# TencentARC/ViT-Lens

Measured on AMD Instinct MI355X. Metric: modality-pairs/sec (ViT-L, 224^2 patches), higher is better.
Workload: dtype bf16; 1 GPU; C3: ViT-L Lens(depth)->ViT + image + text tri-modal InfoNCE TRAINING step (fwd+bwd+AdamW), batch 1024/GPU in micro-batches of 256, first 4 blocks + adapter trainable; global_batch=1024, residual_dtype=bf16, accumulate=fp32, parallelism=dp1, gemm_cfg=-1, via=step, text_tower_operands=fp16, layernorm=folded into the GEMMs (frozen blocks), frozen_towers=second HIP stream beside the trainable tower's forward, backward=two halves of the micro-batches on two HIP streams

## Files before the change

include/vitlens_hip.h:

```cpp
#ifndef VITLENS_HIP_H
#define VITLENS_HIP_H

#include <stdint.h>

#ifdef __cplusplus
extern "C" {
#endif

#ifndef __HIP_PLATFORM_AMD__
typedef struct ihipStream_t* hipStream_t;
#endif

#define VL_EPI_BF16 0
#define VL_EPI_F32 1
#define VL_EPI_RES_F32 2
#define VL_EPI_RES_BF16 3
#define VL_EPI_GEGLU 5
#define VL_EPI_DGELU 6
#define VL_EPI_DGEGLU 7
#define VL_ACT_NONE 0
#define VL_ACT_GELU 1
#define VL_ACT_RELU 2
#define VL_ACT_GELU_DSAVE 4

#define VL_F32 0
#define VL_BF16 1
#define VL_F16 2

#define VL_GEMM_AUTO (-1)
#define VL_GEMM_PERSIST 8
#define VL_GEMM_PINGPONG 10

const char* vl_last_error(void);
#define VL_ABI_VERSION 601
int vl_version(void);

int vl_gemm_bf16(const void* A, const void* W, const float* bias, void* out, const void* res,
                 int M, int N, int K, int lda, int ldw, int ldo, float alpha, int epi, int act,
                 int cfg, hipStream_t stream);

int vl_gemm_splitk_accum_f32(const void* A, const void* W, float* out, int M, int N, int K, int lda, int ldw, long ldo,
                             float alpha, int splits, float* ws, hipStream_t stream);
int vl_gemm_tn_splitk_accum_f32(const void* At, const void* Bt, float* out, int M, int N, int K, int lda, int ldb, long ldo,
                                float alpha, int splits, float* ws, hipStream_t stream);
int vl_gemm_bf16_ex(const void* A, const void* W, const float* bias, void* out, const void* res, void* out2,
                    int M, int N, int K, int lda, int ldw, int ldo, float alpha, int epi, int act,
                    int res_div, int cfg, hipStream_t stream);

int vl_gemm_f16(const void* A, const void* W, const float* bias, void* out, const void* res, int M, int N, int K,
                int lda, int ldw, int ldo, float alpha, int epi, int act, hipStream_t stream);
int vl_attn_fwd_f16(const void* q, const void* k, const void* v, const long* strides, void* out, float* lse,
                    int B, int H, int Lq, int Lk, int dh, float qscale, int causal, hipStream_t stream);

int vl_gemm_f32(const float* A, const float* W, const float* bias, float* out, const float* res, int M, int N, int K,
                int lda, int ldw, int ldo, float alpha, int act, hipStream_t stream);
int vl_attn_fwd_f32(const float* q, const float* k, const float* v, const long* strides, float* out, float* lse,
                    int B, int H, int Lq, int Lk, int dh, float scale, int causal, hipStream_t stream);
int vl_im2col_f32(const float* x, float* patches, int N, int C, int H, int W, int kh, int kw, int sh, int sw,
                  int Kp, int transpose_hw, hipStream_t stream);

int vl_device_info(int device, char* arch, int arch_len, int* cus, int* clock_khz, long* hbm_bytes);

int vl_attn_fwd_bf16(const void* q, const void* k, const void* v, const long* strides, void* out, float* lse,
                     int B, int H, int Lq, int Lk, int dh, float qscale, int causal, hipStream_t stream);

int vl_gemm_main_rows(int M, int N);
int vl_gemm_lnfold_bf16(const void* A, const void* Wg, const float* bias_f, const float* ln_c, const float* ln_mean,
                        const float* ln_rstd, void* out, void* out2, int M, int N, int K, int lda, int ldw, int ldo, int act,
                        hipStream_t stream);
int vl_gemm_res_rowstats_bf16(const void* A, const void* W, const float* bias, void* out, const void* res, float* row_part,
                              int M, int N, int K, int lda, int ldw, int ldo, hipStream_t stream);
int vl_ln_row_stats(const float* row_part, int P, const void* x_bf16, long x_row_stride, int D, int m_main, int rows, float eps,
                    float* mean, float* rstd, const float* ln_w, const float* ln_b, void* y_left, long y_row_stride, int y_row0,
                    hipStream_t stream);

int vl_layernorm_fwd(const void* x, int x_dtype, long x_row_stride, const int64_t* row_index, long row_mul,
                     const float* w, const float* b, void* y, int y_dtype, long y_row_stride,
                     float* mean, float* rstd, int rows, int D, float eps, hipStream_t stream);

int vl_assemble_ln_pre(const void* tokens, int tok_dtype, const float* cls, const float* pos, const float* pos2,
// ... 114 lines not shown
```

vit-lens_amd/csrc/vl_gemm.hip:

```cpp
#include "vl_gemm_common.h"

namespace {

template <int EPI, int MT, int NTL>
__device__ __forceinline__ void store_tile(const GemmP& p, f32x16 (&acc)[MT][NTL], int mrow0, int ncol0, int fr, int fg) {
#pragma unroll
  for (int i = 0; i < MT; ++i) {
    const int m = mrow0 + i * 32 + fr;
    if (m >= p.M) continue;
#pragma unroll
    for (int j = 0; j < NTL; ++j) {
#pragma unroll
      for (int q = 0; q < 4; ++q) {
        const int n = ncol0 + j * 32 + q * 8 + fg * 4;
        if (n >= p.N) continue;
        float v[4];
#pragma unroll
        for (int e = 0; e < 4; ++e) v[e] = acc[i][j][q * 4 + e] * p.alpha;
        if (p.bias) {
          const f32x4 bv = *(const f32x4*)(p.bias + n);
#pragma unroll
          for (int e = 0; e < 4; ++e) v[e] += bv[e];
        }
        if constexpr (EPI == EPI_BF16) {
// ... 598 lines not shown
  }
}

static int query_cus() {
  int dev = 0, n = 0;
  if (hipGetDevice(&dev) != hipSuccess || hipDeviceGetAttribute(&n, hipDeviceAttributeMultiprocessorCount, dev) != hipSuccess || n <= 0) n = 256;
  return n;
}
static int num_cus() {
  static const int n = query_cus();
  return n;
}

template <int EPI, int BN = 256, int NWAVES = 8>
hipError_t launch_persist(const GemmP& p, hipStream_t s) {
  using S = Smem<256, BN>;
  constexpr int WM = NWAVES == 4 ? 2 : (BN == 256 ? 2 : 4), WN = NWAVES / WM;
  const int tiles = ((p.M + 255) / 256) * ((p.N + BN - 1) / BN);
  auto kern = gemm_nt_persist2_kernel<256, BN, WM, WN, EPI>;
  constexpr int smem = 2 * S::STAGE + 8 * 4096;
  static const hipError_t attr = hipFuncSetAttribute((const void*)kern, hipFuncAttributeMaxDynamicSharedMemorySize, smem);
  if (attr != hipSuccess) return attr;
  int G = num_cus() & ~7;
  if (tiles < G) G = (tiles + 7) & ~7;
  hipLaunchKernelGGL(kern, dim3(G), dim3(NWAVES * 64), smem, s, p);
  return hipGetLastError();
}

}
bool vl_gemm_park_supported(int epi, const void* params);
int vl_gemm_park_launch(int epi, const void* params, int ncu, hipStream_t s);
bool vl_gemm_pp_supported(int epi, const void* params);
int vl_gemm_pp_launch(int epi, const void* params, int ncu, hipStream_t s);
namespace {

template <int EPI>
hipError_t launch_best_persist(const GemmP& p0, hipStream_t s) {
  const GemmP& p = p0;
  if (vl_gemm_park_supported(EPI, &p)) return (hipError_t)vl_gemm_park_launch(EPI, &p, num_cus(), s);
  if (vl_gemm_pp_supported(EPI, &p)) return (hipError_t)vl_gemm_pp_launch(EPI, &p, num_cus(), s);
  return launch_persist<EPI>(p, s);
}

template <int EPI>
hipError_t dispatch(const GemmP& p, int cfg, hipStream_t s) {
  if (cfg == 8) {
    if (!vl_gemm_park_supported(EPI, &p)) return hipErrorInvalidValue;
    return (hipError_t)vl_gemm_park_launch(EPI, &p, num_cus(), s);
  }
  if (cfg == 10) {
    if (!vl_gemm_pp_supported(EPI, &p)) return hipErrorInvalidValue;
    return (hipError_t)vl_gemm_pp_launch(EPI, &p, num_cus(), s);
  }
  if (cfg == 4 || cfg == 5) return launch_persist<EPI>(p, s);
  if (cfg == 6) return launch_persist<EPI, 128>(p, s);
  if (cfg == 9) return launch_tail<EPI>(p, s);
  if (cfg == 11) return launch<64, 64, 2, 2, EPI, true>(p, s);
  if (cfg == 12) return launch<128, 64, 2, 2, EPI, true>(p, s);
  switch (cfg & 3) {
    case 0: return launch<256, 256, 2, 4, EPI, true>(p, s);
    case 1: return launch<128, 128, 2, 2, EPI, true>(p, s);
    case 2: return launch<256, 256, 2, 4, EPI, false>(p, s);
    default: return launch<128, 128, 2, 2, EPI, false>(p, s);
  }
}

}

extern "C" int vl_set_error(const char* msg);

static int gcd_i(int a, int b) { while (b) { int t = a % b; a = b; b = t; } return a; }

template <int EPI>
static hipError_t run_gemm(const GemmP& p, int cfg, hipStream_t s) {
  if (cfg >= 0) return dispatch<EPI>(p, cfg, s);
  const int G = num_cus() & ~7;
  const int tiles_n = (p.N + 255) / 256, full_m = p.M / 256;
  if ((long)full_m * tiles_n < (G * 3) / 4) return dispatch<EPI>(p, 1, s);
  int step = G / gcd_i(G, tiles_n);
  int main_m = (full_m / step) * step;
  if ((p.N & 255) == 128) {
    step = 2 * G / gcd_i(2 * G, p.N >> 7);
    main_m = (full_m / step) * step;
    if (main_m == 0) main_m = full_m;
  }
  if (main_m == 0) main_m = full_m;
  if (main_m == 0) return launch_persist<EPI>(p, s);
  const int rows_main = main_m * 256;
  GemmP pm = p; pm.M = rows_main;
  hipError_t e = launch_best_persist<EPI>(pm, s);
  if (e != hipSuccess || rows_main == p.M) return e;
  GemmP pr = p;
  pr.M = p.M - rows_main; pr.m_off = p.m_off + rows_main;
  pr.A = p.A + (size_t)rows_main * p.lda;
  constexpr size_t osz = (EPI == EPI_F32 || EPI == EPI_RES_F32) ? 4 : 2;
  if (p.out) pr.out = (unsigned char*)p.out + (size_t)rows_main * p.ldo * osz;
  if (p.res && EPI != EPI_RES_BF16) pr.res = (const unsigned char*)p.res + (size_t)rows_main * p.ldo * osz;
  if (p.out2) pr.out2 = (bf16_t*)p.out2 + (size_t)rows_main * p.ldo * (EPI == EPI_GEGLU ? 2 : 1);
  if (pr.M > 512) return dispatch<EPI>(pr, 1, s);
  const long t64 = (long)((pr.M + 63) / 64) * ((pr.N + 63) / 64);
  return t64 >= 192 ? dispatch<EPI>(pr, 11, s) : launch_tail<EPI>(pr, s);
}

#define VL_CHECK_ARG(c, msg) do { if (!(c)) return vl_set_error(msg); } while (0)

extern "C" int vl_gemm_main_rows(int M, int N) {
  const int G = num_cus() & ~7;
  if (M <= 0 || N <= 0 || (N & 255)) return 0;
  const int tiles_n = N / 256, full_m = M / 256;
  if ((long)full_m * tiles_n < (G * 3) / 4) return 0;
  const int step = G / gcd_i(G, tiles_n);
  int main_m = (full_m / step) * step;
  if (main_m == 0) main_m = full_m;
  return main_m * 256;
}

extern "C" int vl_gemm_lnfold_bf16(const void* A, const void* Wg, const float* bias_f, const float* ln_c, const float* ln_mean,
                                   const float* ln_rstd, void* out, void* out2, int M, int N, int K, int lda, int ldw, int ldo,
                                   int act, hipStream_t stream) {
  VL_CHECK_ARG(A && Wg && bias_f && ln_c && ln_mean && ln_rstd && out, "vl_gemm_lnfold_bf16: null operand");
  VL_CHECK_ARG(act == VL_ACT_NONE || act == VL_ACT_GELU || act == VL_ACT_GELU_DSAVE, "vl_gemm_lnfold_bf16: act must be none, GELU or GELU_DSAVE");
  VL_CHECK_ARG((act == VL_ACT_GELU_DSAVE) == (out2 != nullptr), "vl_gemm_lnfold_bf16: out2 goes with VL_ACT_GELU_DSAVE");
  VL_CHECK_ARG((((uintptr_t)ln_c | (uintptr_t)bias_f) & 15) == 0, "vl_gemm_lnfold_bf16: column vectors must be 16-byte aligned");
  GemmP p{};
  p.A = (const bf16_t*)A; p.W = (const bf16_t*)Wg; p.bias = bias_f; p.out = out; p.out2 = out2;
  p.M = M; p.N = N; p.K = K; p.lda = lda; p.ldw = ldw; p.ldo = ldo; p.alpha = 1.0f; p.act = act; p.res_div = 1;
  p.ln_mean = ln_mean; p.ln_rstd = ln_rstd; p.ln_c = ln_c;
  const GemmP& q = p;
  VL_CHECK_ARG(vl_gemm_park_supported(EPI_BF16, &q), "vl_gemm_lnfold_bf16: whole 256x256 tiles, K >= 512, 16-byte aligned operands required");
  const hipError_t e = (hipError_t)vl_gemm_park_launch(EPI_BF16, &q, num_cus(), stream);
  if (e != hipSuccess) return vl_set_error(hipGetErrorString(e));
  return 0;
}

extern "C" int vl_gemm_res_rowstats_bf16(const void* A, const void* W, const float* bias, void* out, const void* res,
                                         float* row_part, int M, int N, int K, int lda, int ldw, int ldo, hipStream_t stream) {
  VL_CHECK_ARG(A && W && out && res && row_part, "vl_gemm_res_rowstats_bf16: null operand");
  VL_CHECK_ARG((((uintptr_t)row_part) & 7) == 0, "vl_gemm_res_rowstats_bf16: row_part must be 8-byte aligned");
  GemmP p{};
  p.A = (const bf16_t*)A; p.W = (const bf16_t*)W; p.bias = bias; p.out = out; p.res = res;
  p.M = M; p.N = N; p.K = K; p.lda = lda; p.ldw = ldw; p.ldo = ldo; p.alpha = 1.0f; p.res_div = 1;
  p.row_part = row_part;
  const GemmP& q = p;
  VL_CHECK_ARG(vl_gemm_park_supported(EPI_RES_BF16, &q), "vl_gemm_res_rowstats_bf16: whole 256x256 tiles, K >= 512, 16-byte aligned operands required");
  const hipError_t e = (hipError_t)vl_gemm_park_launch(EPI_RES_BF16, &q, num_cus(), stream);
  if (e != hipSuccess) return vl_set_error(hipGetErrorString(e));
  return 0;
}

extern "C" int vl_gemm_bf16_ex(const void* A, const void* W, const float* bias, void* out, const void* res, void* out2,
                               int M, int N, int K, int lda, int ldw, int ldo, float alpha, int epi, int act,
                               int res_div, int cfg, hipStream_t stream);
extern "C" int vl_gemm_bf16(const void* A, const void* W, const float* bias, void* out, const void* res,
                            int M, int N, int K, int lda, int ldw, int ldo, float alpha, int epi, int act,
                            int cfg, hipStream_t stream) {
  return vl_gemm_bf16_ex(A, W, bias, out, res, nullptr, M, N, K, lda, ldw, ldo, alpha, epi, act, 1, cfg, stream);
}

extern "C" int vl_gemm_bf16_ex(const void* A, const void* W, const float* bias, void* out, const void* res, void* out2,
                               int M, int N, int K, int lda, int ldw, int ldo, float alpha, int epi, int act,
                               int res_div, int cfg, hipStream_t stream) {
  VL_CHECK_ARG(res_div >= 1, "vl_gemm_bf16: res_div must be >= 1");
  VL_CHECK_ARG(res_div == 1 || epi == VL_EPI_RES_BF16, "vl_gemm_bf16: row-broadcast residual needs VL_EPI_RES_BF16");
  VL_CHECK_ARG(M > 0 && N > 0 && K > 0, "vl_gemm_bf16: empty problem");
  VL_CHECK_ARG((K & 63) == 0, "vl_gemm_bf16: K must be a multiple of 64");
  VL_CHECK_ARG((N & 3) == 0, "vl_gemm_bf16: N must be a multiple of 4");
  VL_CHECK_ARG((lda & 7) == 0 && (ldw & 7) == 0, "vl_gemm_bf16: lda/ldw must be multiples of 8");
  VL_CHECK_ARG((ldo & 3) == 0, "vl_gemm_bf16: ldo must be a multiple of 4");
  GemmP p{};
  p.A = (const bf16_t*)A; p.W = (const bf16_t*)W; p.bias = bias; p.out = out; p.res = res; p.out2 = out2;
  p.M = M; p.N = N; p.K = K; p.lda = lda; p.ldw = ldw; p.ldo = ldo; p.alpha = alpha; p.act = act; p.res_div = res_div;
  hipError_t e;
  switch (epi) {
    case VL_EPI_BF16:
      VL_CHECK_ARG(act != VL_ACT_GELU_DSAVE || out2, "vl_gemm_bf16: VL_ACT_GELU_DSAVE needs out2 (the gelu' tensor)");
      e = run_gemm<EPI_BF16>(p, cfg, stream); break;
    case VL_EPI_F32: e = run_gemm<EPI_F32>(p, cfg, stream); break;
    case VL_EPI_RES_F32: VL_CHECK_ARG(res, "vl_gemm_bf16: residual missing"); e = run_gemm<EPI_RES_F32>(p, cfg, stream); break;
    case VL_EPI_RES_BF16: VL_CHECK_ARG(res, "vl_gemm_bf16: residual missing"); e = run_gemm<EPI_RES_BF16>(p, cfg, stream); break;
    case VL_EPI_GEGLU: e = run_gemm<EPI_GEGLU>(p, cfg, stream); break;
    case VL_EPI_DGELU: VL_CHECK_ARG(res, "vl_gemm_bf16: pre-activation tensor missing"); e = run_gemm<EPI_DGELU>(p, cfg, stream); break;
    case VL_EPI_DGEGLU: VL_CHECK_ARG(res, "vl_gemm_bf16: pre-activation tensor missing"); VL_CHECK_ARG((ldo & 7) == 0, "vl_gemm_bf16: DGEGLU needs ldo % 8 == 0"); e = run_gemm<EPI_DGEGLU>(p, cfg, stream); break;
    default: return vl_set_error("vl_gemm_bf16: unknown epilogue");
  }
  if (e != hipSuccess) return vl_set_error(hipGetErrorString(e));
  return 0;
}

extern "C" int vl_gemm_f16(const void* A, const void* W, const float* bias, void* out, const void* res, int M, int N, int K,
                           int lda, int ldw, int ldo, float alpha, int epi, int act, hipStream_t stream) {
  VL_CHECK_ARG(A && W && out, "vl_gemm_f16: null operand");
  VL_CHECK_ARG(epi == VL_EPI_BF16 || epi == VL_EPI_RES_F32, "vl_gemm_f16: VL_EPI_BF16 (16-bit output, here fp16) or VL_EPI_RES_F32");
  VL_CHECK_ARG(epi != VL_EPI_RES_F32 || (res && act == VL_ACT_NONE), "vl_gemm_f16: VL_EPI_RES_F32 needs res and takes no activation");
  VL_CHECK_ARG(act == VL_ACT_NONE || act == VL_ACT_GELU, "vl_gemm_f16: act must be none or GELU");
  GemmP p{};
  p.A = (const bf16_t*)A; p.W = (const bf16_t*)W; p.bias = bias; p.out = out; p.res = res;
  p.M = M; p.N = N; p.K = K; p.lda = lda; p.ldw = ldw; p.ldo = ldo; p.alpha = alpha; p.act = act; p.res_div = 1; p.f16 = 1;
  const int e_ = epi == VL_EPI_BF16 ? (int)EPI_BF16 : (int)EPI_RES_F32;
  VL_CHECK_ARG(vl_gemm_park_supported(e_, &p), "vl_gemm_f16: whole 256x256 tiles (M % 256 == N % 256 == 0), K % 64 == 0, K >= 512, 16-byte aligned operands required");
  const hipError_t e = (hipError_t)vl_gemm_park_launch(e_, &p, num_cus(), stream);
  if (e != hipSuccess) return vl_set_error(hipGetErrorString(e));
  return 0;
}

bool vl_gemm_tn_supported(const void* params);
int vl_gemm_tn_launch(const void* params, int ncu, hipStream_t s);

extern "C" int vl_gemm_tn_splitk_accum_f32(const void* At, const void* Bt, float* out, int M, int N, int K, int lda, int ldb,
                                           long ldo, float alpha, int splits, float* ws, hipStream_t stream) {
  VL_CHECK_ARG(M > 0 && N > 0 && K > 0, "vl_gemm_tn_splitk: empty problem");
  VL_CHECK_ARG((M & 255) == 0 && (N & 255) == 0 && (K & 63) == 0, "vl_gemm_tn_splitk: M % 256, N % 256, K % 64 required");
  VL_CHECK_ARG((lda & 7) == 0 && (ldb & 7) == 0 && (ldo & 3) == 0 && lda >= M && ldb >= N, "vl_gemm_tn_splitk: lda/ldb % 8, ldo % 4, lda >= M, ldb >= N required");
  VL_CHECK_ARG(splits >= 1 && splits <= 1024 && ws, "vl_gemm_tn_splitk: 1 <= splits <= 1024 and a workspace of splits*M*N floats");
  const int nk = K >> 6;
  const int len = (nk + splits - 1) / splits, eff = (nk + len - 1) / len;
// ... 52 lines not shown
```

vit-lens_amd/vitlens_hip/_lib.py:

```python
import ctypes as C
import os

_HERE = os.path.dirname(os.path.abspath(__file__))
_LIB = None


class LibraryNotBuilt(ImportError):
    pass


def lib_path() -> str:
    return os.path.join(_HERE, "libvitlens_hip.so")


P, I, L, F = C.c_void_p, C.c_int, C.c_long, C.c_float

ABI_VERSION = 601

SIGNATURES = {
    "vl_version": [],
    "vl_device_info": [I, C.c_char_p, I, C.POINTER(I), C.POINTER(I), C.POINTER(L)],
    "vl_gemm_bf16": [P, P, P, P, P, I, I, I, I, I, I, F, I, I, I, P],
    "vl_gemm_splitk_accum_f32": [P, P, P, I, I, I, I, I, L, F, I, P, P],
    "vl_gemm_tn_splitk_accum_f32": [P, P, P, I, I, I, I, I, L, F, I, P, P],
    "vl_attn_fwd_bf16": [P, P, P, P, P, P, I, I, I, I, I, F, I, P],
    "vl_gemm_f16": [P, P, P, P, P, I, I, I, I, I, I, F, I, I, P],
    "vl_gemm_f32": [P, P, P, P, P, I, I, I, I, I, I, F, I, P],
    "vl_attn_fwd_f32": [P, P, P, P, P, P, I, I, I, I, I, F, I, P],
    "vl_im2col_f32": [P, P, I, I, I, I, I, I, I, I, I, I, P],
    "vl_attn_fwd_f16": [P, P, P, P, P, P, I, I, I, I, I, F, I, P],
    "vl_layernorm_fwd": [P, I, L, P, L, P, P, P, I, L, P, P, I, I, F, P],
    "vl_gemm_main_rows": [I, I],
    "vl_gemm_lnfold_bf16": [P, P, P, P, P, P, P, P, I, I, I, I, I, I, I, P],
    "vl_gemm_res_rowstats_bf16": [P, P, P, P, P, P, I, I, I, I, I, I, P],
    "vl_ln_row_stats": [P, I, P, L, I, I, I, F, P, P, P, P, P, L, I, P],
    "vl_assemble_ln_pre": [P, I, P, P, P, P, P, P, I, P, P, P, I, I, I, F, P],
    "vl_l2_normalize": [P, P, P, P, I, I, F, P],
    "vl_l2_normalize_bwd": [P, P, P, P, I, I, F, P],
    "vl_im2col_bf16": [P, P, I, I, I, I, I, I, I, I, I, I, P],
    "vl_text_embed": [P, P, P, P, I, I, I, I, I, P],
    "vl_cast_f32_bf16": [P, P, L, P],
    "vl_add_rows": [P, I, P, P, I, L, I, I, P],
    "vl_transpose_to_bf16": [P, I, L, I, I, P, L, P],
    "vl_transpose_colsum_bf16": [P, I, L, I, I, P, L, P, F, P, P],
    "vl_split_bf16x3": [P, P, L, I, I, P],
    "vl_ce_stats": [P, L, I, I, I, P, P, P, P, P],
    "vl_ce_loss_accum": [P, P, P, I, I, I, F, F, P, P],
    "vl_ce_grad": [P, L, I, I, I, P, P, F, F, P, L, P, L, F, P, P, P],
    "vl_ce_grad_ws_floats": [I, I, L, L],
    "vl_gemm_bf16_ex": [P, P, P, P, P, P, I, I, I, I, I, I, F, I, I, I, I, P],
    "vl_kaldi_fbank": [P, L, I, L, P, P, P, I, I, I, I, I, F, F, F, P],
    "vl_fps": [P, P, P, P, I, I, I, P],
    "vl_pc_gather_normalize": [P, P, P, I, I, I, I, P],
    "vl_resample_h_u8": [P, L, I, I, I, I, P, P, I, I, I, P, P],
    "vl_resample_v_u8_norm": [P, I, I, I, I, P, P, I, I, I, P, P, P, P, P],
    "vl_resample_batch_u8_norm": [P, I, I, I, I, I, P, P, P, P, P, P],
    "vl_resample_h_f32": [P, L, I, I, I, P, P, I, I, I, I, F, F, F, P, P],
    "vl_resample_v_f32_norm": [P, I, I, I, P, P, I, I, I, F, F, P, P],
    "vl_knn_group": [P, P, P, P, I, I, I, I, I, P],
    "vl_ball_group": [P, P, P, P, P, I, I, I, I, F, I, I, P],
    "vl_group_max": [P, L, P, I, L, L, I, I, P],
    "vl_pad3_bf16": [P, P, L, I, P],
    "vl_bn_stats": [P, L, I, I, P, I, P, P, P, P, F, P],
    "vl_bn_stats_local": [P, L, I, I, P, I, P, P],
    "vl_bn_stats_merge": [P, I, I, P, P, P, P, F, P, P],
    "vl_bn_bwd_reduce": [P, L, P, L, P, P, P, P, F, I, P, I, P, P, P, I, I, P],
    "vl_bn_bwd_apply": [P, L, P, L, P, P, P, P, F, I, P, P, P, L, I, I, P],
    "vl_bn_apply": [P, L, P, P, P, P, F, I, P, L, L, I, P],
    "vl_bn_bwd": [P, L, P, L, P, P, P, P, F, I, I, P, I, P, P, P, L, I, I, P],
    "vl_group_max_bwd": [P, L, P, L, P, L, P, L, L, I, I, P],
    "vl_group_sum": [P, L, P, L, L, I, I, P],
    "vl_layernorm_bwd": [P, I, L, P, I, L, P, P, P, P, P, P, L, I, I, P],
    "vl_layernorm_bwd_g": [P, I, L, P, I, L, P, P, P, P, P, I, P, L, I, I, P],
    "vl_colreduce_ws_floats": [I, I, I],
    "vl_layernorm_bwd_params": [P, I, L, P, I, L, P, P, P, P, I, I, P, P],
    "vl_colsum": [P, I, L, P, I, I, F, P, P],
    "vl_gelu_bf16": [P, P, L, P],
    "vl_geglu_bf16": [P, P, L, I, P],
    "vl_attn_bwd_bf16": [P, P, P, P, P, P, P, P, P, P, P, L, L, I, I, I, I, I, F, I, F, P],
    "vl_attn_bwd_fused_supported": [I, I, I, I],
    "vl_attn_bwd_fused_bf16": [P, P, P, P, P, P, P, P, P, P, L, L, I, I, I, I, F, F, P],
    "vl_adamw_step": [P, P, P, P, L, F, F, F, F, F, I, F, P],
    "vl_clamp_scalar": [P, F, F, P],
    "vl_axpy_f32": [P, P, F, L, P],
    "vl_scale_exp_f32": [P, P, L, P, F, P],
    "vl_batch_rowsum": [P, P, I, I, I, L, L, P],
    "vl_comm_unique_id": [P],
    "vl_comm_create": [C.POINTER(P), P, I, I],
    "vl_comm_destroy": [P],
    "vl_allgather_embed": [P, P, P, L, P],
    "vl_reducescatter_grad": [P, P, P, L, P],
    "vl_allreduce_grad": [P, P, L, P],
}


_RET = {"vl_colreduce_ws_floats": L, "vl_ce_grad_ws_floats": L}


def load_library():
    global _LIB
    if _LIB is not None:
        return _LIB
    path = lib_path()
    if not os.path.exists(path):
        raise LibraryNotBuilt(
            f"{path} is missing: build it with `python -c 'import __graft_entry__ as g; g.build()'` "
            "or `make -C vit-lens_amd/csrc` (hipcc --offload-arch=gfx950). No CPU/eager fallback exists.")
    lib = C.CDLL(path)
    lib.vl_last_error.restype = C.c_char_p
    lib.vl_last_error.argtypes = []
    for name, args in SIGNATURES.items():
        fn = getattr(lib, name)
        fn.argtypes = args
        fn.restype = _RET.get(name, I)
    got = int(lib.vl_version())
    if got != ABI_VERSION:
        raise RuntimeError(f"{path} reports ABI version {got}, this binding was written for {ABI_VERSION} "
                           "(include/vitlens_hip.h: VL_ABI_VERSION): rebuild the library (`make -C vit-lens_amd/csrc`)")
    _LIB = lib
    return lib


def check(status: int):
    if status != 0:
        raise RuntimeError("libvitlens_hip: " + load_library().vl_last_error().decode())
```

vit-lens_amd/vitlens_hip/ops.py:

```python
import ctypes as C
import threading

import torch

from ._lib import load_library, check

F32, BF16, F16 = 0, 1, 2
EPI_BF16, EPI_F32, EPI_RES_F32, EPI_RES_BF16, EPI_GEGLU, EPI_DGELU, EPI_DGEGLU = 0, 1, 2, 3, 5, 6, 7
ACT_NONE, ACT_GELU, ACT_RELU = 0, 1, 2
ACT_GELU_DSAVE = 4
LOG2E = 1.4426950408889634

_lib = load_library()


def _stream():
    return C.c_void_p(torch.cuda.current_stream().cuda_stream)


def _p(t):
    if t is None:
        return None
    if not t.is_cuda:
        raise RuntimeError("vitlens_hip ops need GPU tensors (no CPU fallback)")
# ... 14 lines not shown
    if t.dim() != 2 or t.stride(1) != 1:
        raise ValueError(f"{name}: need a row-major 2-D tensor, got shape {tuple(t.shape)} strides {t.stride()}")
    if dtype is not None and t.dtype != dtype:
        raise TypeError(f"{name}: expected {dtype}, got {t.dtype}")


def gemm(a, w, bias=None, out=None, res=None, epi=EPI_BF16, act=ACT_NONE, alpha=1.0, cfg=-1, out2=None, res_div=1):
    if act == ACT_GELU_DSAVE and epi == EPI_BF16 and out2 is None:
        raise ValueError("gemm: ACT_GELU_DSAVE needs out2")
    _chk2d(a, "a", torch.bfloat16); _chk2d(w, "w", torch.bfloat16)
    M, K = a.shape
    N = w.shape[0]
    if w.shape[1] != K:
        raise ValueError(f"gemm: K mismatch {a.shape} vs {w.shape}")
    if K % 64:
        Kp = (K + 63) // 64 * 64
        a = torch.nn.functional.pad(a, (0, Kp - K)); w = torch.nn.functional.pad(w, (0, Kp - K))
        K = Kp
    if out is None:
        n_out = N // 2 if epi == EPI_GEGLU else (2 * N if epi == EPI_DGEGLU else N)
        odt = torch.float32 if epi in (EPI_F32, EPI_RES_F32) else torch.bfloat16
        out = torch.empty(M, n_out, device=a.device, dtype=odt)
    _chk2d(out, "out")
    if res is not None:
        _chk2d(res, "res")
        if res.stride(0) != out.stride(0) or res.dtype != out.dtype:
            raise ValueError("gemm: residual must share out's row stride and dtype")
        if res_div > 1 and res.shape[0] * res_div < M:
            raise ValueError("gemm: broadcast residual has too few rows")
    if bias is not None and (bias.dtype != torch.float32 or bias.numel() != N):
        raise ValueError("gemm: bias must be f32 [N]")
    if out2 is not None and (out2.stride(0) != out.stride(0) * (2 if epi == EPI_GEGLU else 1) or out2.dtype != torch.bfloat16):
        raise ValueError("gemm: out2 must be bf16 with out's row stride (twice that for GEGLU)")
    check(_lib.vl_gemm_bf16_ex(_p(a), _p(w), _p(bias), _p(out), _p(res), _p(out2), M, N, K, a.stride(0), w.stride(0),
                               out.stride(0), float(alpha), epi, act, res_div, cfg, _stream()))
    return out


def gemm_f16(a, w, bias=None, out=None, res=None, epi=EPI_BF16, act=ACT_NONE, alpha=1.0):
    _chk2d(a, "a", torch.float16); _chk2d(w, "w", torch.float16)
    M, K = a.shape
    N = w.shape[0]
    if w.shape[1] != K:
        raise ValueError(f"gemm_f16: K mismatch {a.shape} vs {w.shape}")
    if out is None:
        out = torch.empty(M, N, device=a.device, dtype=torch.float32 if epi == EPI_RES_F32 else torch.float16)
    _chk2d(out, "out", torch.float32 if epi == EPI_RES_F32 else torch.float16)
    if res is not None:
        _chk2d(res, "res", torch.float32)
        if res.stride(0) != out.stride(0):
            raise ValueError("gemm_f16: residual must share out's row stride")
    if bias is not None and (bias.dtype != torch.float32 or bias.numel() != N):
        raise ValueError("gemm_f16: bias must be f32 [N]")
    check(_lib.vl_gemm_f16(_p(a), _p(w), _p(bias), _p(out), _p(res), M, N, K, a.stride(0), w.stride(0), out.stride(0),
                           float(alpha), epi, act, _stream()))
    return out


def gemm_f32(a, w, bias=None, out=None, res=None, act=ACT_NONE, alpha=1.0):
    _chk2d(a, "a", torch.float32); _chk2d(w, "w", torch.float32)
    M, K = a.shape
    N = w.shape[0]
    if w.shape[1] != K:
        raise ValueError(f"gemm_f32: K mismatch {a.shape} vs {w.shape}")
    if out is None:
        out = torch.empty(M, N, device=a.device, dtype=torch.float32)
    _chk2d(out, "out", torch.float32)
    if res is not None:
        _chk2d(res, "res", torch.float32)
# ... 26 lines not shown
    if x.dtype != torch.float32 or not x.is_contiguous():
        raise ValueError("im2col_f32: need contiguous f32 input")
    N, Cc = x.shape[0], x.shape[1]
    H, W = (x.shape[3], x.shape[2]) if transpose_hw else (x.shape[2], x.shape[3])
    gh, gw = (H - kh) // sh + 1, (W - kw) // sw + 1
    out = torch.empty(N * gh * gw, Kp, device=x.device, dtype=torch.float32)
    check(_lib.vl_im2col_f32(_p(x), _p(out), N, Cc, H, W, kh, kw, sh, sw, Kp, 1 if transpose_hw else 0, _stream()))
    return out, gh, gw


def fold_ln_linear(w, b, gamma, beta):
    w = w.detach().float()
    wg = (w * gamma.detach().float()[None, :]).to(torch.bfloat16).contiguous()
    c = wg.float().sum(1).contiguous()
    d = (b.detach().float() + (w * beta.detach().float()[None, :]).sum(1)).contiguous()
    return wg, d, c


def _fold_rows(x, out, N, K):
    M = x.shape[0]
    if x.dtype != torch.bfloat16 or out.dtype != torch.bfloat16 or K < 512 or K % 64 or N % 256 or x.stride(0) % 8 or out.stride(0) % 8:
        return 0
    if x.data_ptr() % 16 or out.data_ptr() % 16:
        return 0
    return int(_lib.vl_gemm_main_rows(M, N))


def _leftover_cfg(rows, N, cfg):
    if cfg >= 0 or rows > 512:
        return cfg
    return 11 if ((rows + 63) // 64) * ((N + 63) // 64) >= 192 else 9


def gemm_lnfold(x, fold, mean, rstd, out, w, b, ln_w, ln_b, h_ws, act=ACT_NONE, out2=None, eps=1e-5, cfg=-1, h_ready=False):
    wg, d, c = fold
    M, K = x.shape
    N = wg.shape[0]
    mm = _fold_rows(x, out, N, K)
    if mm:
        check(_lib.vl_gemm_lnfold_bf16(_p(x), _p(wg), _p(d), _p(c), _p(mean), _p(rstd), _p(out), _p(out2), mm, N, K,
                                       x.stride(0), wg.stride(0), out.stride(0), act, _stream()))
    if mm < M:
        r = M - mm
        h = h_ws[:r]
        if not h_ready:
            layernorm(x[mm:], ln_w, ln_b, h, r, K, x_row_stride=x.stride(0), mean=mean[mm:], rstd=rstd[mm:], eps=eps)
        gemm(h, w, b, out=out[mm:], epi=EPI_BF16, act=act, cfg=_leftover_cfg(r, N, cfg) if mm else cfg,
             out2=None if out2 is None else out2[mm:])
    return out


def gemm_res_rowstats(a, w, b, out, res, part, cfg=-1):
    M, K = a.shape
    N = w.shape[0]
    mm = _fold_rows(a, out, N, K) if (res.dtype == torch.bfloat16 and res.stride(0) == out.stride(0) and res.data_ptr() % 16 == 0
                                      and part.numel() >= M * (N // 64) * 2) else 0
    if mm:
        check(_lib.vl_gemm_res_rowstats_bf16(_p(a), _p(w), _p(b), _p(out), _p(res), _p(part), mm, N, K, a.stride(0), w.stride(0),
                                             out.stride(0), _stream()))
    if mm < M:
        gemm(a[mm:], w, b, out=out[mm:], res=res[mm:], epi=EPI_RES_BF16, cfg=_leftover_cfg(M - mm, N, cfg) if mm else cfg)
    return mm


def fold_rows(x, out, N):
    return _fold_rows(x, out, N, x.shape[1])


def ln_row_stats(part, x, m_main, mean, rstd, eps=1e-5, ln_w=None, ln_b=None, h_left=None, h_row0=None):
    rows, D = x.shape
    if h_left is not None:
        if h_row0 is None or h_row0 < m_main or h_left.dtype != torch.bfloat16 or h_left.shape[0] < rows - h_row0:
            raise ValueError("ln_row_stats: h_left needs h_row0 >= m_main and a bf16 buffer of at least rows - h_row0 rows")
    check(_lib.vl_ln_row_stats(_p(part) if m_main else None, D // 64, _p(x), x.stride(0), D, m_main, rows, float(eps), _p(mean),
                               _p(rstd), _p(ln_w), _p(ln_b), _p(h_left), h_left.stride(0) if h_left is not None else 0,
                               int(h_row0 or 0), _stream()))


def logits_gemm(xb, yb, scale):
    Cn = yb.shape[0]
    Cp = (Cn + 3) // 4 * 4
    if Cp != Cn:
        yb = torch.cat([yb, torch.zeros(Cp - Cn, yb.shape[1], device=yb.device, dtype=yb.dtype)], 0)
    out = gemm(xb, yb, None, epi=EPI_F32, alpha=scale)
    return out if Cp == Cn else out[:, :Cn]


def gemm_dw(dyt, xt, g, cfg=-1, alpha=1.0):
    _chk2d(dyt, "dyt", torch.bfloat16); _chk2d(xt, "xt", torch.bfloat16); _chk2d(g, "g", torch.float32)
    M, K = dyt.shape
    N = xt.shape[0]
    nk = K // 64
    if K % 64 == 0 and M % 256 == 0 and N % 256 == 0 and nk >= 64:
        t256 = (M // 256) * (N // 256)
# ... 492 lines not shown
```

Baseline: 1772 modality-pairs/sec.

## Add split-K 64x64 leftover GEMM kernel with workspace-based partial reduction

```diff
diff --git a/include/vitlens_hip.h b/include/vitlens_hip.h
--- a/include/vitlens_hip.h
+++ b/include/vitlens_hip.h
@@ -32,7 +32,7 @@
 #define VL_GEMM_PINGPONG 10
 
 const char* vl_last_error(void);
-#define VL_ABI_VERSION 601
+#define VL_ABI_VERSION 602
 int vl_version(void);
 
 int vl_gemm_bf16(const void* A, const void* W, const float* bias, void* out, const void* res,
@@ -46,6 +46,10 @@
 int vl_gemm_bf16_ex(const void* A, const void* W, const float* bias, void* out, const void* res, void* out2,
                     int M, int N, int K, int lda, int ldw, int ldo, float alpha, int epi, int act,
                     int res_div, int cfg, hipStream_t stream);
+int vl_gemm_bf16_ws(const void* A, const void* W, const float* bias, void* out, const void* res, void* out2,
+                    int M, int N, int K, int lda, int ldw, int ldo, float alpha, int epi, int act,
+                    int res_div, int cfg, void* ws, hipStream_t stream);
+long vl_gemm_ws_bytes(void);
 
 int vl_gemm_f16(const void* A, const void* W, const float* bias, void* out, const void* res, int M, int N, int K,
                 int lda, int ldw, int ldo, float alpha, int epi, int act, hipStream_t stream);
diff --git a/vit-lens_amd/csrc/vl_gemm.hip b/vit-lens_amd/csrc/vl_gemm.hip
--- a/vit-lens_amd/csrc/vl_gemm.hip
+++ b/vit-lens_amd/csrc/vl_gemm.hip
@@ -654,6 +654,10 @@
 int vl_gemm_park_launch(int epi, const void* params, int ncu, hipStream_t s);
 bool vl_gemm_pp_supported(int epi, const void* params);
 int vl_gemm_pp_launch(int epi, const void* params, int ncu, hipStream_t s);
+size_t vl_gemm_left_ws_bytes();
+bool vl_gemm_left_supported(int epi, const void* params);
+bool vl_gemm_left_preferred(const void* params);
+int vl_gemm_left_launch(int epi, const void* params, void* ws, int slices, hipStream_t s);
 namespace {
 
 template <int EPI>
@@ -694,7 +698,11 @@
 static int gcd_i(int a, int b) { while (b) { int t = a % b; a = b; b = t; } return a; }
 
 template <int EPI>
-static hipError_t run_gemm(const GemmP& p, int cfg, hipStream_t s) {
+static hipError_t run_gemm(const GemmP& p, int cfg, void* ws, hipStream_t s) {
+  if (cfg >= 0 && (cfg & 255) == 13) {
+    if (!ws || !vl_gemm_left_supported(EPI, &p)) return hipErrorInvalidValue;
+    return (hipError_t)vl_gemm_left_launch(EPI, &p, ws, cfg >> 8, s);
+  }
   if (cfg >= 0) return dispatch<EPI>(p, cfg, s);
   const int G = num_cus() & ~7;
   const int tiles_n = (p.N + 255) / 256, full_m = p.M / 256;
@@ -720,6 +728,7 @@
   if (p.res && EPI != EPI_RES_BF16) pr.res = (const unsigned char*)p.res + (size_t)rows_main * p.ldo * osz;
   if (p.out2) pr.out2 = (bf16_t*)p.out2 + (size_t)rows_main * p.ldo * (EPI == EPI_GEGLU ? 2 : 1);
   if (pr.M > 512) return dispatch<EPI>(pr, 1, s);
+  if (ws && vl_gemm_left_supported(EPI, &pr) && vl_gemm_left_preferred(&pr)) return (hipError_t)vl_gemm_left_launch(EPI, &pr, ws, 0, s);
   const long t64 = (long)((pr.M + 63) / 64) * ((pr.N + 63) / 64);
   return t64 >= 192 ? dispatch<EPI>(pr, 11, s) : launch_tail<EPI>(pr, s);
 }
@@ -779,9 +788,21 @@
   return vl_gemm_bf16_ex(A, W, bias, out, res, nullptr, M, N, K, lda, ldw, ldo, alpha, epi, act, 1, cfg, stream);
 }
 
+extern "C" int vl_gemm_bf16_ws(const void* A, const void* W, const float* bias, void* out, const void* res, void* out2,
+                               int M, int N, int K, int lda, int ldw, int ldo, float alpha, int epi, int act,
+                               int res_div, int cfg, void* ws, hipStream_t stream);
 extern "C" int vl_gemm_bf16_ex(const void* A, const void* W, const float* bias, void* out, const void* res, void* out2,
                                int M, int N, int K, int lda, int ldw, int ldo, float alpha, int epi, int act,
                                int res_div, int cfg, hipStream_t stream) {
+  return vl_gemm_bf16_ws(A, W, bias, out, res, out2, M, N, K, lda, ldw, ldo, alpha, epi, act, res_div, cfg, nullptr, stream);
+}
+
+extern "C" long vl_gemm_ws_bytes(void) { return (long)vl_gemm_left_ws_bytes(); }
+
+extern "C" int vl_gemm_bf16_ws(const void* A, const void* W, const float* bias, void* out, const void* res, void* out2,
+                               int M, int N, int K, int lda, int ldw, int ldo, float alpha, int epi, int act,
+                               int res_div, int cfg, void* ws, hipStream_t stream) {
+  VL_CHECK_ARG((((uintptr_t)ws) & 15) == 0, "vl_gemm_bf16: ws must be 16-byte aligned");
   VL_CHECK_ARG(res_div >= 1, "vl_gemm_bf16: res_div must be >= 1");
   VL_CHECK_ARG(res_div == 1 || epi == VL_EPI_RES_BF16, "vl_gemm_bf16: row-broadcast residual needs VL_EPI_RES_BF16");
   VL_CHECK_ARG(M > 0 && N > 0 && K > 0, "vl_gemm_bf16: empty problem");
@@ -796,13 +817,13 @@
   switch (epi) {
     case VL_EPI_BF16:
       VL_CHECK_ARG(act != VL_ACT_GELU_DSAVE || out2, "vl_gemm_bf16: VL_ACT_GELU_DSAVE needs out2 (the gelu' tensor)");
-      e = run_gemm<EPI_BF16>(p, cfg, stream); break;
-    case VL_EPI_F32: e = run_gemm<EPI_F32>(p, cfg, stream); break;
-    case VL_EPI_RES_F32: VL_CHECK_ARG(res, "vl_gemm_bf16: residual missing"); e = run_gemm<EPI_RES_F32>(p, cfg, stream); break;
-    case VL_EPI_RES_BF16: VL_CHECK_ARG(res, "vl_gemm_bf16: residual missing"); e = run_gemm<EPI_RES_BF16>(p, cfg, stream); break;
-    case VL_EPI_GEGLU: e = run_gemm<EPI_GEGLU>(p, cfg, stream); break;
-    case VL_EPI_DGELU: VL_CHECK_ARG(res, "vl_gemm_bf16: pre-activation tensor missing"); e = run_gemm<EPI_DGELU>(p, cfg, stream); break;
-    case VL_EPI_DGEGLU: VL_CHECK_ARG(res, "vl_gemm_bf16: pre-activation tensor missing"); VL_CHECK_ARG((ldo & 7) == 0, "vl_gemm_bf16: DGEGLU needs ldo % 8 == 0"); e = run_gemm<EPI_DGEGLU>(p, cfg, stream); break;
+      e = run_gemm<EPI_BF16>(p, cfg, ws, stream); break;
+    case VL_EPI_F32: e = run_gemm<EPI_F32>(p, cfg, ws, stream); break;
+    case VL_EPI_RES_F32: VL_CHECK_ARG(res, "vl_gemm_bf16: residual missing"); e = run_gemm<EPI_RES_F32>(p, cfg, ws, stream); break;
+    case VL_EPI_RES_BF16: VL_CHECK_ARG(res, "vl_gemm_bf16: residual missing"); e = run_gemm<EPI_RES_BF16>(p, cfg, ws, stream); break;
+    case VL_EPI_GEGLU: e = run_gemm<EPI_GEGLU>(p, cfg, ws, stream); break;
+    case VL_EPI_DGELU: VL_CHECK_ARG(res, "vl_gemm_bf16: pre-activation tensor missing"); e = run_gemm<EPI_DGELU>(p, cfg, ws, stream); break;
+    case VL_EPI_DGEGLU: VL_CHECK_ARG(res, "vl_gemm_bf16: pre-activation tensor missing"); VL_CHECK_ARG((ldo & 7) == 0, "vl_gemm_bf16: DGEGLU needs ldo % 8 == 0"); e = run_gemm<EPI_DGEGLU>(p, cfg, ws, stream); break;
     default: return vl_set_error("vl_gemm_bf16: unknown epilogue");
   }
   if (e != hipSuccess) return vl_set_error(hipGetErrorString(e));
diff --git a/vit-lens_amd/csrc/vl_gemm_left.hip b/vit-lens_amd/csrc/vl_gemm_left.hip
--- /dev/null
+++ b/vit-lens_amd/csrc/vl_gemm_left.hip
@@ -0,0 +1,247 @@
+#include "vl_gemm_common.h"
+
+namespace {
+
+constexpr int LF_STAGE = 65536;
+constexpr int LF_LDS = 2 * LF_STAGE;
+constexpr int LF_MAX_TILES = 1024;
+constexpr size_t LF_CNT_BYTES = 4096;
+constexpr size_t LF_WS_BYTES = LF_CNT_BYTES + (size_t)LF_MAX_TILES * 64 * 64 * 4;
+
+typedef __attribute__((address_space(3))) void* lf_lds_t;
+
+template <int EPI>
+__global__ void __launch_bounds__(256) gemm_left_kernel(const GemmP p, unsigned* __restrict__ cnt, float* __restrict__ part) {
+  extern __shared__ __attribute__((aligned(16))) unsigned char smem[];
+  const int tiles_m = (p.M + 63) >> 6;
+  const int nk = p.K >> 6;
+  const int L = p.ksplit_len;
+  const int S = (nk + L - 1) / L;
+  const int tile = blockIdx.x / S, sl = blockIdx.x - tile * S;
+  const int tn = tile / tiles_m, tm = tile - tn * tiles_m;
+  const int m0 = tm << 6, n0 = tn << 6;
+  const int kb0 = sl * L, kb1 = min(kb0 + L, nk);
+
+  const int tid = threadIdx.x, lane = tid & 63;
+  const int wid = __builtin_amdgcn_readfirstlane(tid >> 6);
+  const int wave_m = wid & 1, wave_n = wid >> 1;
+
+  __amdgpu_buffer_rsrc_t rsA = __builtin_amdgcn_make_buffer_rsrc((void*)(p.A + (size_t)kb0 * 64), 0, 0x7ffffff0, 0x00020000);
+  __amdgpu_buffer_rsrc_t rsW = __builtin_amdgcn_make_buffer_rsrc((void*)(p.W + (size_t)kb0 * 64), 0, 0x7ffffff0, 0x00020000);
+  unsigned voffA[2], voffW[2];
+#pragma unroll
+  for (int u = 0; u < 2; ++u) {
+    const int r = u * 32 + wid * 8 + (lane >> 3);
+    const int sw = ((lane & 7) ^ ((r >> 1) & 7)) * 16;
+    const int gm = min(m0 + r, p.M - 1), gn = min(n0 + r, p.N - 1);
+    voffA[u] = (unsigned)(gm * p.lda * 2 + sw);
+    voffW[u] = (unsigned)(gn * p.ldw * 2 + sw);
+  }
+
+  const int fr16 = lane & 15, fq = lane >> 4;
+  const int fsw = (fr16 >> 1) & 7;
+  const int fa = (wave_m * 32 + fr16) * 128, fw = 32768 + (wave_n * 32 + fr16) * 128;
+  f32x4 acc[2][2];
+#pragma unroll
+  for (int i = 0; i < 2; ++i)
+#pragma unroll
+    for (int j = 0; j < 2; ++j) acc[i][j] = f32x4{0.f, 0.f, 0.f, 0.f};
+
+  auto dma_chunk = [&](int c0, unsigned char* stage) {
+    const int nb = min(4, kb1 - c0);
+    for (int b = 0; b < nb; ++b) {
+      const int soff = (c0 - kb0 + b) * 128;
+#pragma unroll
+      for (int u = 0; u < 2; ++u) {
+        __builtin_amdgcn_raw_ptr_buffer_load_lds(rsA, (lf_lds_t)(stage + b * 8192 + (u * 4 + wid) * 1024), 16, voffA[u], soff, 0, 0);
+        __builtin_amdgcn_raw_ptr_buffer_load_lds(rsW, (lf_lds_t)(stage + 32768 + b * 8192 + (u * 4 + wid) * 1024), 16, voffW[u], soff, 0, 0);
+      }
+    }
+  };
+  dma_chunk(kb0, smem);
+  int par = 0;
+  for (int c0 = kb0; c0 < kb1; c0 += 4) {
+    const int nb = min(4, kb1 - c0);
+    const int nxt = min(4, max(0, kb1 - c0 - 4));
+    unsigned char* const cur = smem + par * LF_STAGE;
+    if (nxt) dma_chunk(c0 + 4, smem + (par ^ 1) * LF_STAGE);
+    switch (nxt) {
+      case 0: asm volatile("s_waitcnt vmcnt(0)\n\ts_barrier" ::: "memory"); break;
+      case 1: asm volatile("s_waitcnt vmcnt(4)\n\ts_barrier" ::: "memory"); break;
+      case 2: asm volatile("s_waitcnt vmcnt(8)\n\ts_barrier" ::: "memory"); break;
+      case 3: asm volatile("s_waitcnt vmcnt(12)\n\ts_barrier" ::: "memory"); break;
+      default: asm volatile("s_waitcnt vmcnt(16)\n\ts_barrier" ::: "memory"); break;
+    }
+    for (int b = 0; b < nb; ++b) {
+#pragma unroll
+      for (int h = 0; h < 2; ++h) {
+        const int off = b * 8192 + ((h * 4 + fq) ^ fsw) * 16;
+        bf16x8 af[2], wf[2];
+#pragma unroll
+        for (int i = 0; i < 2; ++i) af[i] = *(const bf16x8*)(cur + fa + i * 2048 + off);
+#pragma unroll
+        for (int j = 0; j < 2; ++j) wf[j] = *(const bf16x8*)(cur + fw + j * 2048 + off);
+#pragma unroll
+        for (int i = 0; i < 2; ++i)
+#pragma unroll
+          for (int j = 0; j < 2; ++j) acc[i][j] = __builtin_amdgcn_mfma_f32_16x16x32_bf16(wf[j], af[i], acc[i][j], 0, 0, 0);
+      }
+    }
+    asm volatile("s_waitcnt lgkmcnt(0)\n\ts_barrier" ::: "memory");
+    par ^= 1;
+  }
+
+  if (S > 1) {
+    float* const mine = part + (size_t)tile * S * 4096;
+    __amdgpu_buffer_rsrc_t rsP = __builtin_amdgcn_make_buffer_rsrc((void*)(mine + (size_t)sl * 4096), 0, 0x7ffffff0, 0x00020000);
+#pragma unroll
+    for (int i = 0; i < 2; ++i)
+#pragma unroll
+      for (int j = 0; j < 2; ++j)
+        __builtin_amdgcn_raw_buffer_store_b128(__builtin_bit_cast(u32x4, acc[i][j]), rsP, (((wid * 2 + i) * 2 + j) * 64 + lane) * 16, 0, 16);
+    asm volatile("s_waitcnt vmcnt(0)" ::: "memory");
+    __syncthreads();
+    if (tid == 0) {
+      const unsigned old = __hip_atomic_fetch_add(cnt + tile, 1u, __ATOMIC_RELAXED, __HIP_MEMORY_SCOPE_AGENT);
+      const int last = old == (unsigned)(S - 1);
+      if (last) __hip_atomic_store(cnt + tile, 0u, __ATOMIC_RELAXED, __HIP_MEMORY_SCOPE_AGENT);
+      *(volatile int*)smem = last;
+    }
+    __syncthreads();
+    if (!*(volatile int*)smem) return;
+    __amdgpu_buffer_rsrc_t rsR = __builtin_amdgcn_make_buffer_rsrc((void*)mine, 0, 0x7ffffff0, 0x00020000);
+    const int lo = (wid * 4 * 64 + lane) * 16;
+#pragma unroll
+    for (int i = 0; i < 2; ++i)
+#pragma unroll
+      for (int j = 0; j < 2; ++j) acc[i][j] = __builtin_bit_cast(f32x4, __builtin_amdgcn_raw_buffer_load_b128(rsR, lo + (i * 2 + j) * 1024, 0, 16));
+    for (int s = 1; s < S; ++s) {
+      f32x4 t[2][2];
+#pragma unroll
+      for (int i = 0; i < 2; ++i)
+#pragma unroll
+        for (int j = 0; j < 2; ++j)
+          t[i][j] = __builtin_bit_cast(f32x4, __builtin_amdgcn_raw_buffer_load_b128(rsR, s * 16384 + lo + (i * 2 + j) * 1024, 0, 16));
+#pragma unroll
+      for (int i = 0; i < 2; ++i)
+#pragma unroll
+        for (int j = 0; j < 2; ++j) acc[i][j] += t[i][j];
+    }
+  }
+
+  mfma_results_settled();
+#pragma unroll
+  for (int j = 0; j < 2; ++j) {
+    const int n = n0 + wave_n * 32 + j * 16 + fq * 4;
+    if (n >= p.N) continue;
+    const f32x4 bv = p.bias ? *(const f32x4*)(p.bias + n) : f32x4{0.f, 0.f, 0.f, 0.f};
+#pragma unroll
+    for (int i = 0; i < 2; ++i) {
+      const int m = m0 + wave_m * 32 + i * 16 + fr16;
+      if (m >= p.M) continue;
+      f32x4 v = scale_bias(acc[i][j], p.alpha, bv);
+      const size_t o = (size_t)m * p.ldo + n;
+      u32x2 w;
+      if constexpr (EPI == EPI_BF16) {
+        if (p.act == 1 && !p.out2) {
+#pragma unroll
+          for (int e = 0; e < 4; e += 2) { const vl_f32x2 y = gelu_erf2(vl_f32x2{v[e], v[e + 1]}); v[e] = y[0]; v[e + 1] = y[1]; }
+        } else if (p.act == 2) {
+#pragma unroll
+          for (int e = 0; e < 4; ++e) v[e] = fmaxf(v[e], 0.f);
+        }
+        w[0] = pack2bf(v[0], v[1]); w[1] = pack2bf(v[2], v[3]);
+        if (p.act == 1 && p.out2) {
+          *(u32x2*)((bf16_t*)p.out2 + o) = w;
+#pragma unroll
+          for (int e = 0; e < 2; ++e) w[e] = pack2bf(gelu_erf2(unpack2bf(w[e])));
+        } else if (p.act == 4) {
+          u32x2 d;
+#pragma unroll
+          for (int e = 0; e < 2; ++e) { unsigned int y, g; gelu_and_grad_pk(w[e], y, g); w[e] = y; d[e] = g; }
+          *(u32x2*)((bf16_t*)p.out2 + o) = d;
+        }
+      } else if constexpr (EPI == EPI_RES_BF16) {
+        const u32x2 rr = *(const u32x2*)((const bf16_t*)p.res + (size_t)((m + p.m_off) / p.res_div) * p.ldo + n);
+#pragma unroll
+        for (int e = 0; e < 2; ++e) {
+          const vl_f32x2 x = unpack2bf(pack2bf(v[2 * e], v[2 * e + 1])) + unpack2bf(rr[e]);
+          w[e] = p.act == 2 ? pack2bf(fmaxf(x[0], 0.f), fmaxf(x[1], 0.f)) : pack2bf(x);
+        }
+      } else {
+        const u32x2 rr = *(const u32x2*)((const bf16_t*)p.res + o);
+#pragma unroll
+        for (int e = 0; e < 2; ++e) {
+          const unsigned int x = pack2bf(v[2 * e], v[2 * e + 1]);
+          w[e] = p.act == 4 ? mul_pk_bf16(x, rr[e]) : pack2bf(unpack2bf(x) * gelu_erf_grad2(unpack2bf(rr[e])));
+        }
+      }
+      *(u32x2*)((bf16_t*)p.out + o) = w;
+    }
+  }
+}
+
+static int left_slices(int tiles, int nk) {
+  return max(1, min(256 / tiles, nk / 12));
+}
+
+template <int EPI>
+hipError_t launch_left(const GemmP& p0, void* ws, int slices, hipStream_t s) {
+  GemmP p = p0;
+  const int tiles = ((p.M + 63) >> 6) * ((p.N + 63) >> 6);
+  const int nk = p.K >> 6;
+  if (slices <= 0) slices = left_slices(tiles, nk);
+  slices = min(min(slices, nk), LF_MAX_TILES / tiles);
+  p.ksplit_len = (nk + slices - 1) / slices;
+  const int S = (nk + p.ksplit_len - 1) / p.ksplit_len;
+  auto kern = gemm_left_kernel<EPI>;
+  static const hipError_t attr = hipFuncSetAttribute((const void*)kern, hipFuncAttributeMaxDynamicSharedMemorySize, LF_LDS);
+  if (attr != hipSuccess) return attr;
+  unsigned* cnt = (unsigned*)ws;
+  float* part = (float*)((unsigned char*)ws + LF_CNT_BYTES);
+  hipLaunchKernelGGL(kern, dim3(tiles * S), dim3(256), LF_LDS, s, p, cnt, part);
+  return hipGetLastError();
+}
+
+}
+
+size_t vl_gemm_left_ws_bytes() { return LF_WS_BYTES; }
+
+bool vl_gemm_left_preferred(const void* params) {
+  const GemmP& p = *(const GemmP*)params;
+  const int tiles = ((p.M + 63) >> 6) * ((p.N + 63) >> 6);
+  return !(left_slices(tiles, p.K >> 6) == 1 && tiles < 128);
+}
+
+bool vl_gemm_left_supported(int epi, const void* params) {
+  const GemmP& p = *(const GemmP*)params;
+  if (p.M <= 0 || p.M > 512 || p.N <= 0 || (p.N & 3) || p.K <= 0 || (p.K & 63) || p.f16 || p.ln_mean || p.row_part) return false;
+  if (((p.M + 63) >> 6) * ((p.N + 63) >> 6) > LF_MAX_TILES) return false;
+  if (epi == EPI_BF16) {
+    if (!(p.act == 0 || p.act == 1 || p.act == 2 || p.act == 4)) return false;
+    if (p.act == 4 && !p.out2) return false;
+    if (p.out2 && p.act != 1 && p.act != 4) return false;
+  } else if (epi == EPI_RES_BF16) {
+    if (!p.res || p.res_div < 1 || !(p.act == 0 || p.act == 2)) return false;
+  } else if (epi == EPI_DGELU) {
+    if (!p.res || !(p.act == 0 || p.act == 4)) return false;
+  } else {
+    return false;
+  }
+  if ((p.lda & 7) || (p.ldw & 7) || (p.ldo & 3)) return false;
+  if (((uintptr_t)p.A | (uintptr_t)p.W) & 15) return false;
+  if (((uintptr_t)p.out | (uintptr_t)p.res | (uintptr_t)p.out2) & 7) return false;
+  if ((long)(p.M - 1) * p.lda * 2 + (long)p.K * 2 >= 0x7ffffff0L || (long)(p.N - 1) * p.ldw * 2 + (long)p.K * 2 >= 0x7ffffff0L) return false;
+  return true;
+}
+
+int vl_gemm_left_launch(int epi, const void* params, void* ws, int slices, hipStream_t s) {
+  const GemmP& p = *(const GemmP*)params;
+  if (!ws) return (int)hipErrorInvalidValue;
+  switch (epi) {
+    case EPI_BF16: return (int)launch_left<EPI_BF16>(p, ws, slices, s);
+    case EPI_RES_BF16: return (int)launch_left<EPI_RES_BF16>(p, ws, slices, s);
+    case EPI_DGELU: return (int)launch_left<EPI_DGELU>(p, ws, slices, s);
+    default: return (int)hipErrorInvalidValue;
+  }
+}
diff --git a/vit-lens_amd/vitlens_hip/_lib.py b/vit-lens_amd/vitlens_hip/_lib.py
--- a/vit-lens_amd/vitlens_hip/_lib.py
+++ b/vit-lens_amd/vitlens_hip/_lib.py
@@ -15,7 +15,7 @@
 
 P, I, L, F = C.c_void_p, C.c_int, C.c_long, C.c_float
 
-ABI_VERSION = 601
+ABI_VERSION = 602
 
 SIGNATURES = {
     "vl_version": [],
@@ -49,6 +49,8 @@
     "vl_ce_grad": [P, L, I, I, I, P, P, F, F, P, L, P, L, F, P, P, P],
     "vl_ce_grad_ws_floats": [I, I, L, L],
     "vl_gemm_bf16_ex": [P, P, P, P, P, P, I, I, I, I, I, I, F, I, I, I, I, P],
+    "vl_gemm_bf16_ws": [P, P, P, P, P, P, I, I, I, I, I, I, F, I, I, I, I, P, P],
+    "vl_gemm_ws_bytes": [],
     "vl_kaldi_fbank": [P, L, I, L, P, P, P, I, I, I, I, I, F, F, F, P],
     "vl_fps": [P, P, P, P, I, I, I, P],
     "vl_pc_gather_normalize": [P, P, P, I, I, I, I, P],
@@ -94,7 +96,7 @@
 }
 
 
-_RET = {"vl_colreduce_ws_floats": L, "vl_ce_grad_ws_floats": L}
+_RET = {"vl_colreduce_ws_floats": L, "vl_ce_grad_ws_floats": L, "vl_gemm_ws_bytes": L}
 
 
 def load_library():
diff --git a/vit-lens_amd/vitlens_hip/ops.py b/vit-lens_amd/vitlens_hip/ops.py
--- a/vit-lens_amd/vitlens_hip/ops.py
+++ b/vit-lens_amd/vitlens_hip/ops.py
@@ -70,9 +70,23 @@
         raise ValueError("gemm: bias must be f32 [N]")
     if out2 is not None and (out2.stride(0) != out.stride(0) * (2 if epi == EPI_GEGLU else 1) or out2.dtype != torch.bfloat16):
         raise ValueError("gemm: out2 must be bf16 with out's row stride (twice that for GEGLU)")
-    check(_lib.vl_gemm_bf16_ex(_p(a), _p(w), _p(bias), _p(out), _p(res), _p(out2), M, N, K, a.stride(0), w.stride(0),
-                               out.stride(0), float(alpha), epi, act, res_div, cfg, _stream()))
-    return out
+    stream = torch.cuda.current_stream().cuda_stream
+    ws = _gemm_ws(a.device, stream) if cfg == -1 or cfg % 256 == 13 else None
+    check(_lib.vl_gemm_bf16_ws(_p(a), _p(w), _p(bias), _p(out), _p(res), _p(out2), M, N, K, a.stride(0), w.stride(0),
+                               out.stride(0), float(alpha), epi, act, res_div, cfg, _p(ws), C.c_void_p(stream)))
+    return out
+
+
+_gemm_ws_cache = {}
+
+
+def _gemm_ws(device, stream):
+    key = (device, stream, threading.get_ident())
+    t = _gemm_ws_cache.get(key)
+    if t is None:
+        t = torch.zeros(int(_lib.vl_gemm_ws_bytes()) // 4, device=device, dtype=torch.int32)
+        _gemm_ws_cache[key] = t
+    return t
 
 
 def gemm_f16(a, w, bias=None, out=None, res=None, epi=EPI_BF16, act=ACT_NONE, alpha=1.0):
@@ -165,6 +179,14 @@
     return 11 if ((rows + 63) // 64) * ((N + 63) // 64) >= 192 else 9
 
 
+def _leftover_route(rows, N, K, cfg):
+    if cfg >= 0 or rows > 512:
+        return cfg
+    tiles = ((rows + 63) // 64) * ((N + 63) // 64)
+    slices = max(1, min(256 // tiles, K // 64 // 12))
+    return 9 if slices == 1 and tiles < 128 else 13
+
+
 def gemm_lnfold(x, fold, mean, rstd, out, w, b, ln_w, ln_b, h_ws, act=ACT_NONE, out2=None, eps=1e-5, cfg=-1, h_ready=False):
     wg, d, c = fold
     M, K = x.shape
@@ -178,7 +200,7 @@
         h = h_ws[:r]
         if not h_ready:
             layernorm(x[mm:], ln_w, ln_b, h, r, K, x_row_stride=x.stride(0), mean=mean[mm:], rstd=rstd[mm:], eps=eps)
-        gemm(h, w, b, out=out[mm:], epi=EPI_BF16, act=act, cfg=_leftover_cfg(r, N, cfg) if mm else cfg,
+        gemm(h, w, b, out=out[mm:], epi=EPI_BF16, act=act, cfg=_leftover_route(r, N, K, cfg) if mm else cfg,
              out2=None if out2 is None else out2[mm:])
     return out
 
@@ -192,7 +214,7 @@
         check(_lib.vl_gemm_res_rowstats_bf16(_p(a), _p(w), _p(b), _p(out), _p(res), _p(part), mm, N, K, a.stride(0), w.stride(0),
                                              out.stride(0), _stream()))
     if mm < M:
-        gemm(a[mm:], w, b, out=out[mm:], res=res[mm:], epi=EPI_RES_BF16, cfg=_leftover_cfg(M - mm, N, cfg) if mm else cfg)
+        gemm(a[mm:], w, b, out=out[mm:], res=res[mm:], epi=EPI_RES_BF16, cfg=_leftover_route(M - mm, N, K, cfg) if mm else cfg)
     return mm
 
 
```

Result: no change. 1782 modality-pairs/sec, median of 6 (+0.6%).
